# farhiongit/aho-corasick-1975

Hardware: AMD Instinct MI355X
Metric: input GB/s scanned, 1k-keyword dictionary, bit-exact match set (higher is better)
Workload: dtype u8; 1 GPU; BASELINE configs[1]: 1000 ASCII keywords, 1024 MiB synthetic text per GPU (1073741824 symbols of 1 B), 1 keyword planted per 4096 symbols; states=6492, lmax=12, matches_per_gpu=555000, matches_total=555000, parallelism=text sharded x1, 0-symbol halo (the largest any rank used), tables replicated

## Files before the change

aho-corasick-1975_amd/csrc/dev_gram2.h:

```cpp
constexpr uint32_t G2_STAGE = WAVE * 16 + 16;
constexpr uint32_t G2_LIST = 128;
constexpr uint32_t G2_Q2 = 64;
constexpr uint32_t G2_WAVE_BYTES = G2_STAGE + G2_LIST * 2 + G2_Q2 * 8;
static_assert (G2_WAVE_BYTES % 16 == 0, "the staged text is written 16 bytes per lane");
constexpr uint32_t G2_LDS_FIXED = (SPARSE_THREADS / WAVE) * G2_WAVE_BYTES + WALK_CTX_BYTES;

__device__ __forceinline__ uint32_t
wave_incl_scan_dpp (uint32_t v) {
  v += (uint32_t)__builtin_amdgcn_update_dpp (0, (int)v, 0x111, 0xf, 0xf, false);
  v += (uint32_t)__builtin_amdgcn_update_dpp (0, (int)v, 0x112, 0xf, 0xf, false);
  v += (uint32_t)__builtin_amdgcn_update_dpp (0, (int)v, 0x114, 0xf, 0xf, false);
  v += (uint32_t)__builtin_amdgcn_update_dpp (0, (int)v, 0x118, 0xf, 0xf, false);
  v += (uint32_t)__builtin_amdgcn_update_dpp (0, (int)v, 0x142, 0xa, 0xf, false);
  v += (uint32_t)__builtin_amdgcn_update_dpp (0, (int)v, 0x143, 0xc, 0xf, false);
  return v;
}

template <bool COUNT_ONLY, bool TILED>
__global__ __launch_bounds__ (SPARSE_THREADS) void
scan_gram2_kernel (GramK K, EmitCtx E, Launch A, const unsigned char *__restrict__ text, uint2 *items, uint32_t region_items,
                   uint32_t *fill, RecHole *holes, uint32_t resume, TileEntry *dir, uint32_t dir_base) {
  (void)items;
  (void)region_items;
  (void)fill;
  extern __shared__ __attribute__ ((aligned (16))) unsigned char smem[];
  constexpr uint32_t WAVES = SPARSE_THREADS / WAVE;
  constexpr uint32_t GROUP = WAVE * 16;
  {
    uint4 *dst = reinterpret_cast<uint4 *> (smem);
    const uint4 *src = reinterpret_cast<const uint4 *> (K.tab2);
    for (uint32_t i = threadIdx.x; i < (K.tab2_words + 3) / 4; i += blockDim.x)
      dst[i] = src[i];
  }
  uint32_t *next_tile = reinterpret_cast<uint32_t *> (smem + K.g2_off + WAVES * G2_WAVE_BYTES);
  StartsK *Ks = reinterpret_cast<StartsK *> (next_tile + 4);
  EmitCtx *Es = reinterpret_cast<EmitCtx *> (reinterpret_cast<unsigned char *> (Ks) + WALK_CTX_K);
  WaveRec *Ws = reinterpret_cast<WaveRec *> (reinterpret_cast<unsigned char *> (Ks) + WALK_CTX_K + WALK_CTX_E);
  if (threadIdx.x == 0) {
    *next_tile = 0;
    StartsK Kc{};
    Kc.srec = K.srec;
    Kc.sedge = K.sedge;
    Kc.remap = K.g4gid;
    Kc.remap_base = K.d5_begin;
    Kc.peek = K.g5peek;
    Kc.peek_packed = K.peek_packed;
    Kc.peek_rel = K.d5_rel;
    Kc.lo = K.lo;
    Kc.span = K.span;
    *Ks = Kc;
    *Es = E;
  }
  __syncthreads ();

  const uint32_t lane = threadIdx.x & (WAVE - 1);
  const uint32_t wib = uniform (threadIdx.x / WAVE);
  const uint32_t stage_off = K.g2_off + wib * G2_WAVE_BYTES;
  const uint32_t list_off = stage_off + G2_STAGE;
  uint2 *q2 = reinterpret_cast<uint2 *> (smem + stage_off + G2_STAGE + G2_LIST * 2);
  const uint32_t wave_id = blockIdx.x * WAVES + wib;
  uint2 *hits = reinterpret_cast<uint2 *> (Ws + wib);
  if (lane == 0) {
    WaveRec w0{};
    if (resume && !COUNT_ONLY && holes) {
      const RecHole h = holes[wave_id];
      if (h.len) {
        const unsigned long long at = ((unsigned long long)h.start_hi << 32) | h.start_lo;
        const unsigned long long base = at + h.len - E.rec_chunk;
        const bool below = base + E.rec_chunk <= E.capacity;
        const bool above = base >= E.capacity && base - E.capacity + E.rec_chunk <= E.spill_slots;
        const uint64_t dst = below ? reinterpret_cast<uint64_t> (&E.records[base]) : (above ? reinterpret_cast<uint64_t> (E.spill + (base - E.capacity)) : 0ull);
        w0.dst_lo = (uint32_t)dst;
        w0.dst_hi = (uint32_t)(dst >> 32);
        w0.base_lo = (uint32_t)base;
        w0.base_hi = (uint32_t)(base >> 32);
        w0.limit = (below || above) ? E.rec_chunk : 0u;
        w0.have = 1;
        w0.pad[0] = E.rec_chunk - h.len;
        w0.pad[1] = 1;
        w0.prev1 = w0.prev2 = NONE;
      }
    }
    if (!w0.have)
      w0.prev1 = w0.prev2 = NONE;
    Ws[wib] = w0;
  }
  const TileShare share (A);
  const uint32_t last_blk = (A.n - 1) / 16;
  uint32_t qn2 = 0;
  unsigned long long counted = 0;
  RecState rs = { 0ull, 0u };
  if (!COUNT_ONLY && resume) {
    rs = rec_state_load (hits);
    counted = uniform (reinterpret_cast<const WaveRec *> (hits)->pad[0]);
  }
  uint32_t it_x = 0, it_y = 0, pk = 0;
  uint2 pend_item = make_uint2 (0, 0), pend_e = make_uint2 (0, 0);
  uint32_t pend_r = 0, pend_n = 0;
  constexpr uint32_t PEND_NEED = 0x80000000u;
  auto lds_word = [&] (uint32_t byte_off) -> uint32_t {
    return *reinterpret_cast<const __attribute__ ((address_space (3))) uint32_t *> (byte_off);
  };
  const uint4 *text16 = reinterpret_cast<const uint4 *> (text);
  auto load_group = [&] (uint32_t g) -> uint4 {
    const uint32_t blk = g * WAVE + lane;
    typedef uint32_t nt_u32x4 __attribute__ ((ext_vector_type (4)));
    const nt_u32x4 v = __builtin_nontemporal_load (reinterpret_cast<const nt_u32x4 *> (text16) + (blk < last_blk ? blk : last_blk));
    return make_uint4 (v.x, v.y, v.z, v.w);
  };
  DIAG (const unsigned long long d_t0 = __builtin_readcyclecounter (); unsigned long long d_top = 0, d_sieve = 0, d_take = 0, d_cwait = 0, d_cons = 0, d_walk = 0, d_steps = 0;)
  auto walk_batch = [&] (uint32_t n_items) {
    DIAG (const unsigned long long d_wk = __builtin_readcyclecounter ();)
    const unsigned long long r = walk_starts<uint8_t, COUNT_ONLY, 2> (Ks, Es, text, q2, qn2, n_items, hits, counted);
    qn2 = uniform ((uint32_t)(r >> 32));
    counted = (uint32_t)r;
    if (!COUNT_ONLY)
      rs = rec_state_load (hits);
    DIAG (d_walk += __builtin_readcyclecounter () - d_wk;)
  };
  uint32_t peek_pos = 0, peek_cls = 0, peek_val = 0, peek_n = 0;
  const bool peek_inline = !COUNT_ONLY && K.peek_packed && K.d5_rel;
  auto push_walk = [&] (bool go, uint32_t ix, uint32_t iy) {
    const uint64_t m = __ballot (go);
    if (m) {
      while (qn2 + (uint32_t)__popcll (m) > G2_Q2)
        walk_batch (qn2 < WAVE ? qn2 : WAVE);
      if (go)
        q2[qn2 + rank_below (m)] = make_uint2 (ix, iy);
      qn2 = uniform (qn2 + (uint32_t)__popcll (m));
#if defined(ACM_GRAM2_ABLATE) && ACM_GRAM2_ABLATE == 2
      qn2 = 0;
#endif
      while (qn2 >= WAVE)
        walk_batch (WAVE);
    }
  };
  auto resolve_peeks = [&] () {
    if (peek_n == 0)
      return;
    const uint32_t ev = peek_val, cls = peek_cls & 31u;
    const uint32_t sym = (ev >> 31) ? GRAM_NO_PEEK : (ev >> 23) & 0xFFu;
    const uint32_t c1 = cls < K.span ? K.lo + cls : 0x100u;
    const bool on = (peek_cls >> 31) != 0 && (sym == GRAM_NO_PEEK || sym == c1);
    peek_n = 0;
    push_walk (on, peek_pos, (ev & 0x7FFFFFu) | WI_RECORD | cls << 24);
  };
  auto consume_pending = [&] () {
    if (pend_n == 0)
      return;
    DIAG (const unsigned long long d_c0 = __builtin_readcyclecounter (); asm volatile ("s_waitcnt vmcnt(0)" ::: "memory"); const unsigned long long d_c1 = __builtin_readcyclecounter (); d_cwait += d_c1 - d_c0; d_steps++; const unsigned long long d_w0 = d_walk;)
    struct { uint32_t x, y; } e = { pend_e.x, pend_e.y };
    const bool valid = lane < pend_n && (pend_r & PEND_NEED) != 0;
    const uint32_t r = pend_r & 0xFFu;
#if defined(ACM_GRAM2_ABLATE) && (ACM_GRAM2_ABLATE == 3 || ACM_GRAM2_ABLATE == 8)
    asm volatile ("" :: "v"(e.x), "v"(e.y));
    pend_n = 0;
    return;
#endif
    const bool far = valid && r >= 7 && (e.x & 0x20000000u) != 0;
    if (__ballot (far)) {
      const uint2 o = K.over2[far ? (e.x & 0x1FFFFFFFu) + (r - 7) : 0u];
      e.x = far ? o.x : e.x;
      e.y = far ? o.y : e.y;
    }
    if (!valid)
      e.x = 0;
    const bool at_record = (e.x & 0x40000000u) != 0;
#if !(defined(ACM_GRAM2_ABLATE) && ACM_GRAM2_ABLATE == 1)
    emit_terminals<COUNT_ONLY, true> (E, (e.x >> 31) != 0 && !at_record && pend_item.x + 3 >= E.emit_from, pend_item.x + 3, e.y, 4u, lane, hits, counted, Es, &rs);
    if (!COUNT_ONLY)
      counted = uniform ((uint32_t)counted);
#endif
    const uint32_t c4 = (pend_item.y >> 20) & 31u, c5 = (pend_item.y >> 25) & 31u;
    const bool child = ((e.x >> c4) & 1u) != 0 && !at_record;
    const uint32_t st5 = e.y + __popc (e.x & ((1u << c4) - 1u));
    if (peek_inline) {
      resolve_peeks ();
      uint32_t pv = 0;
      if (child)
        pv = K.g5peek[st5 - K.d5_begin];
      peek_val = pv;
      peek_pos = pend_item.x + 4;
      peek_cls = c5 | (child ? 0x80000000u : 0u);
      peek_n = __ballot (child) != 0 ? 1u : 0u;
      push_walk (at_record, pend_item.x + 3, e.y | WI_RECORD | c4 << 24);
    } else
      push_walk (child || at_record, at_record ? pend_item.x + 3 : pend_item.x + 4,
                 at_record ? e.y | WI_RECORD | (K.d5_rel ? c4 << 24 : 0u) : (K.d5_rel ? (st5 - K.d5_begin) | c5 << 24 : st5));
    pend_n = 0;
    DIAG (d_cons += (__builtin_readcyclecounter () - d_c1) - (d_walk - d_w0);)
  };
  auto batch_step = [&] (uint32_t n_items) {
    const uint32_t idx = it_y & 0xFFFFFu;
    const uint32_t word = lds_word ((idx >> 4) * 4u);
    consume_pending ();
    const uint32_t sh = (idx & 15u) * 2u;
    const bool need = lane < n_items && ((word >> sh) & 1u) != 0;
    const uint32_t r = __popc (word & 0x55555555u & ((1u << sh) - 1u));
    uint2 e = make_uint2 (0, 0);
#if defined(ACM_GRAM2_ABLATE) && ACM_GRAM2_ABLATE == 8
    if (need)
      e = K.rows2[r < 7 ? r : 7];
#else
    if (need)
      e = K.rows2[(size_t)(idx >> 4) * 8 + (r < 7 ? r : 7)];
#endif
    pend_e = e;
    pend_item = make_uint2 (it_x, it_y);
    pend_r = r | (need ? PEND_NEED : 0u);
    pend_n = n_items;
  };

  auto sieve_group = [&] (const uint4 cur, const uint32_t next_x, const uint32_t next_y, const uint32_t g, uint4 &prefetched, uint32_t &pass_out, uint32_t &my_out) -> uint32_t {
    typedef uint32_t u32x4 __attribute__ ((ext_vector_type (4)));
    typedef uint32_t u32x2 __attribute__ ((ext_vector_type (2)));
    uint32_t t4 = (uint32_t)__builtin_amdgcn_update_dpp ((int)uniform (next_x), (int)cur.x, 0x130, 0xf, 0xf, false);
    const uint32_t t5 = (uint32_t)__builtin_amdgcn_update_dpp ((int)uniform (next_y), (int)cur.y, 0x130, 0xf, 0xf, false);
    asm volatile ("" : "+v"(t4));
    __builtin_amdgcn_sched_barrier (0);
    prefetched = load_group (g + 4);
    const uint32_t t0 = cur.x, t1 = cur.y, t2 = cur.z, t3 = cur.w;
    *reinterpret_cast<__attribute__ ((address_space (3))) u32x4 *> (stage_off + lane * 16u) = u32x4{ t0, t1, t2, t3 };
    if (lane == WAVE - 1)
      *reinterpret_cast<__attribute__ ((address_space (3))) u32x2 *> (stage_off + GROUP) = u32x2{ t4, t5 };
    const uint32_t pos0 = g * GROUP + lane * 16;
    const uint32_t w[5] = { t0, t1, t2, t3, t4 };
#if defined(ACM_GRAM2_ABLATE) && ACM_GRAM2_ABLATE == 7
    asm volatile ("" :: "v"(w[0]), "v"(w[1]), "v"(w[2]), "v"(w[3]), "v"(w[4]));
    pass_out = 0;
    return 0;
#endif
    uint32_t c[20];
#pragma unroll
    for (int j = 0; j < 20; j++) {
      const uint32_t b = (w[j / 4] >> (8 * (j % 4))) & 0xFFu;
      c[j] = min (b - K.lo, K.span);
    }
    if (__builtin_expect (uniform (g * GROUP + GROUP + 20) > A.n, 0)) {
#pragma unroll
      for (int j = 0; j < 20; j++)
        if (pos0 + j >= A.n)
          c[j] = K.span;
    }
    uint32_t pair[19];
#pragma unroll
    for (int j = 0; j < 19; j++)
      pair[j] = __umul24 (c[j], K.W) + c[j + 1];
    const uint32_t W2 = K.W * K.W;
    uint32_t acc = 0;
#pragma unroll
    for (int h = 0; h < 2; h++) {
      uint32_t ix[8], word[8];
#pragma unroll
      for (int j = 0; j < 8; j++) {
        ix[j] = __umul24 (pair[8 * h + j], W2) + pair[8 * h + j + 2];
        word[j] = lds_word ((ix[j] >> 4) * 4u);
      }
#pragma unroll
      for (int j = 0; j < 8; j++)
        acc |= __builtin_amdgcn_ubfe (word[j], ix[j] << 1, 2u) << (2 * (8 * h + j));
    }
    const uint32_t ix16 = __umul24 (pair[16], W2) + pair[18];
    const uint32_t h16 = __builtin_amdgcn_ubfe (lds_word ((ix16 >> 4) * 4u), (ix16 << 1) | 1u, 1u);
    const uint32_t pass = acc & ((acc >> 1) | (acc >> 3) | (h16 << 30)) & 0x55555555u;
    pass_out = pass;
#if defined(ACM_GRAM2_ABLATE) && ACM_GRAM2_ABLATE == 6
    asm volatile ("" :: "v"(pass));
    return 0;
#endif
    const uint32_t cnt = __popc (pass);
    const uint32_t incl = wave_incl_scan_dpp (cnt);
    my_out = incl - cnt;
    return (uint32_t)__builtin_amdgcn_readlane ((int)incl, WAVE - 1);
  };
  auto take_group = [&] (const uint32_t g, const uint32_t total, uint32_t pass, uint32_t my) {
    const uint32_t W2 = K.W * K.W;
    const bool tail = g * GROUP + GROUP + 8 > A.n;
    for (uint32_t base = 0; base < total; base += G2_LIST) {
      const uint32_t n_here = total - base < G2_LIST ? total - base : G2_LIST;
      {
        const uint32_t lim = base + n_here;
        while (pass != 0 && my < lim) {
          const uint32_t b = (uint32_t)__builtin_ctz (pass);
          *reinterpret_cast<__attribute__ ((address_space (3))) uint16_t *> (list_off + (my - base) * 2u) = (uint16_t)(lane * 16u + (b >> 1));
          pass &= pass - 1u;
          my++;
        }
      }
#if defined(ACM_GRAM2_ABLATE) && ACM_GRAM2_ABLATE == 5
      continue;
#endif
      for (uint32_t off = 0; off < n_here;) {
        const uint32_t take = n_here - off < WAVE - pk ? n_here - off : WAVE - pk;
        const bool mine = lane >= pk && lane < pk + take;
        const uint32_t li = mine ? off + lane - pk : 0u;
        const uint32_t q = *reinterpret_cast<const __attribute__ ((address_space (3))) uint16_t *> (list_off + li * 2u);
        const uint32_t a = stage_off + (q & ~3u);
        const uint32_t d0 = lds_word (a), d1 = lds_word (a + 4u), d2 = lds_word (a + 8u);
        const uint32_t lo4 = __builtin_amdgcn_alignbyte (d1, d0, q), hi4 = __builtin_amdgcn_alignbyte (d2, d1, q);
        uint32_t r[6];
#pragma unroll
        for (int k = 0; k < 6; k++) {
          const uint32_t b = ((k < 4 ? lo4 : hi4) >> (8 * (k % 4))) & 0xFFu;
          r[k] = min (b - K.lo, K.span);
        }
        const uint32_t p = g * GROUP + q;
        if (tail) {
#pragma unroll
          for (int k = 0; k < 6; k++)
            if (p + k >= A.n)
              r[k] = K.span;
        }
        const uint32_t idx = __umul24 (__umul24 (r[0], K.W) + r[1], W2) + __umul24 (r[2], K.W) + r[3];
        const uint32_t y = idx | (r[4] << 20) | (r[5] << 25);
        it_x = mine ? p : it_x;
        it_y = mine ? y : it_y;
        pk += take;
        off += take;
#if defined(ACM_GRAM2_ABLATE) && ACM_GRAM2_ABLATE == 4
        if (pk == WAVE) {
          asm volatile ("" :: "v"(it_x), "v"(it_y));
          pk = 0;
        }
        continue;
#endif
        if (pk == WAVE) {
          batch_step (WAVE);
          pk = 0;
        }
      }
    }
  };

  static_assert (!TILED || !COUNT_ONLY, "tiled scans write their records themselves");
  constexpr bool tiled = TILED;
  auto stream_index = [&] (const WaveRec &w) -> uint32_t { return w.have ? (w.pad[1] - 1u) * REC_CHUNK + (uint32_t)counted : 0u; };
  if (tiled && lane == 0)
    Ws[wib].tile = NONE;
  auto drain = [&] () {
    if (pk) {
      batch_step (pk);
      pk = 0;
    }
    consume_pending ();
    resolve_peeks ();
    while (qn2)
      walk_batch (qn2 < WAVE ? qn2 : WAVE);
  };
  for (;;) {
    const uint32_t tile = share.next (next_tile, lane);
    if (tiled) {
      drain ();
      if (lane == 0) {
        const WaveRec w = Ws[wib];
        if (w.tile != NONE) {
          const uint32_t s_end = stream_index (w), cur_tile = w.tile;
          const uint32_t tile_begin = cur_tile * K.R * GROUP, tile_len = K.R * GROUP;
          const uint32_t tile_end = A.n - tile_begin < tile_len ? A.n : tile_begin + tile_len;
          TileEntry e;
          e.end_slot = w.have ? (((unsigned long long)w.base_hi << 32) | w.base_lo) + (uint32_t)counted : 0ull;
          e.lo = E.pos_base + (tile_begin > E.emit_from ? tile_begin : E.emit_from);
          e.hi = E.pos_base + tile_end;
          e.n = s_end - w.s_begin;
          e.n_late = s_end - w.s_late;
          e.c1 = w.prev1;
          e.c2 = w.prev1 != NONE ? w.prev2 : NONE;
          e.pad[0] = e.pad[1] = 0;
          dir[dir_base + (cur_tile - A.range_begin)] = e;
        }
      }
    }
    if (tile == NONE)
      break;
    if (tiled && lane == 0) {
      WaveRec *W = Ws + wib;
      W->tile = tile;
      W->s_begin = W->s_late = stream_index (*W);
    }
    const uint32_t g0 = tile * K.R;
    uint4 c0 = load_group (g0), c1 = load_group (g0 + 1), c2 = load_group (g0 + 2), c3 = load_group (g0 + 3);
    for (uint32_t k = 0; k < K.R; k++) {
      if (tiled && k + 1 == K.R && lane == 0)
        Ws[wib].s_late = stream_index (Ws[wib]);
      uint4 n3;
      uint32_t pass = 0, my = 0;
      DIAG (const unsigned long long d_g0 = __builtin_readcyclecounter (); asm volatile ("s_waitcnt vmcnt(0)" ::: "memory"); const unsigned long long d_g1 = __builtin_readcyclecounter (); d_top += d_g1 - d_g0;)
      const uint32_t total = sieve_group (c0, c1.x, c1.y, g0 + k, n3, pass, my);
      DIAG (const unsigned long long d_g2 = __builtin_readcyclecounter (); d_sieve += d_g2 - d_g1; const unsigned long long d_in = d_cwait + d_cons + d_walk;)
      if (total)
        take_group (g0 + k, total, pass, my);
      DIAG (d_take += (__builtin_readcyclecounter () - d_g2) - (d_cwait + d_cons + d_walk - d_in);)
      c0 = c1;
      c1 = c2;
      c2 = c3;
      c3 = n3;
    }
  }
  if (!tiled)
    drain ();
  DIAG (if (lane == 0 && wave_id < 8192) {
    unsigned long long *o = g_acm_diag[wave_id];
    o[0] = __builtin_readcyclecounter () - d_t0;
    o[1] = d_top;
    o[2] = d_sieve;
    o[3] = d_take;
    o[4] = d_cwait;
    o[5] = d_cons;
    o[6] = d_walk;
    o[7] = d_steps;
  })
  if (COUNT_ONLY) {
    const uint32_t incl = wave_incl_scan ((uint32_t)counted);
    const uint32_t total = __shfl (incl, WAVE - 1, WAVE);
    if (lane == 0 && total)
      atomicAdd (E.count, (unsigned long long)total);
  } else {
    if (lane == 0 && holes) {
      const WaveRec w = Ws[wib];
      const unsigned long long at = (((unsigned long long)w.base_hi << 32) | w.base_lo) + (uint32_t)counted;
      RecHole h = { (uint32_t)at, (uint32_t)(at >> 32), w.have ? E.rec_chunk - (uint32_t)counted : 0u, 0u };
      holes[wave_id] = h;
    }
  }
}
```

Baseline: 3853 GB/s.

## Unroll sieve loop by four with rotating registers and move prefetch after sieve math

```diff
diff --git a/aho-corasick-1975_amd/csrc/dev_gram2.h b/aho-corasick-1975_amd/csrc/dev_gram2.h
--- a/aho-corasick-1975_amd/csrc/dev_gram2.h
+++ b/aho-corasick-1975_amd/csrc/dev_gram2.h
@@ -14,6 +14,13 @@
   v += (uint32_t)__builtin_amdgcn_update_dpp (0, (int)v, 0x142, 0xa, 0xf, false);
   v += (uint32_t)__builtin_amdgcn_update_dpp (0, (int)v, 0x143, 0xc, 0xf, false);
   return v;
+}
+
+__device__ __forceinline__ uint32_t
+mad24 (uint32_t a, uint32_t s, uint32_t c) {
+  uint32_t d;
+  asm ("v_mad_u32_u24 %0, %1, %2, %3" : "=v"(d) : "v"(a), "s"(s), "v"(c));
+  return d;
 }
 
 template <bool COUNT_ONLY, bool TILED>
@@ -98,18 +105,18 @@
   uint2 pend_item = make_uint2 (0, 0), pend_e = make_uint2 (0, 0);
   uint32_t pend_r = 0, pend_n = 0;
   constexpr uint32_t PEND_NEED = 0x80000000u;
-  auto lds_word = [&] (uint32_t byte_off) -> uint32_t {
+  auto lds_word = [&] (uint32_t byte_off) __attribute__ ((always_inline)) -> uint32_t {
     return *reinterpret_cast<const __attribute__ ((address_space (3))) uint32_t *> (byte_off);
   };
   const uint4 *text16 = reinterpret_cast<const uint4 *> (text);
-  auto load_group = [&] (uint32_t g) -> uint4 {
+  auto load_group = [&] (uint32_t g) __attribute__ ((always_inline)) -> uint4 {
     const uint32_t blk = g * WAVE + lane;
     typedef uint32_t nt_u32x4 __attribute__ ((ext_vector_type (4)));
     const nt_u32x4 v = __builtin_nontemporal_load (reinterpret_cast<const nt_u32x4 *> (text16) + (blk < last_blk ? blk : last_blk));
     return make_uint4 (v.x, v.y, v.z, v.w);
   };
   DIAG (const unsigned long long d_t0 = __builtin_readcyclecounter (); unsigned long long d_top = 0, d_sieve = 0, d_take = 0, d_cwait = 0, d_cons = 0, d_walk = 0, d_steps = 0;)
-  auto walk_batch = [&] (uint32_t n_items) {
+  auto walk_batch = [&] (uint32_t n_items) __attribute__ ((always_inline)) {
     DIAG (const unsigned long long d_wk = __builtin_readcyclecounter ();)
     const unsigned long long r = walk_starts<uint8_t, COUNT_ONLY, 2> (Ks, Es, text, q2, qn2, n_items, hits, counted);
     qn2 = uniform ((uint32_t)(r >> 32));
@@ -120,7 +127,7 @@
   };
   uint32_t peek_pos = 0, peek_cls = 0, peek_val = 0, peek_n = 0;
   const bool peek_inline = !COUNT_ONLY && K.peek_packed && K.d5_rel;
-  auto push_walk = [&] (bool go, uint32_t ix, uint32_t iy) {
+  auto push_walk = [&] (bool go, uint32_t ix, uint32_t iy) __attribute__ ((always_inline)) {
     const uint64_t m = __ballot (go);
     if (m) {
       while (qn2 + (uint32_t)__popcll (m) > G2_Q2)
@@ -135,7 +142,7 @@
         walk_batch (WAVE);
     }
   };
-  auto resolve_peeks = [&] () {
+  auto resolve_peeks = [&] () __attribute__ ((always_inline)) {
     if (peek_n == 0)
       return;
     const uint32_t ev = peek_val, cls = peek_cls & 31u;
@@ -145,7 +152,7 @@
     peek_n = 0;
     push_walk (on, peek_pos, (ev & 0x7FFFFFu) | WI_RECORD | cls << 24);
   };
-  auto consume_pending = [&] () {
+  auto consume_pending = [&] () __attribute__ ((always_inline)) {
     if (pend_n == 0)
       return;
     DIAG (const unsigned long long d_c0 = __builtin_readcyclecounter (); asm volatile ("s_waitcnt vmcnt(0)" ::: "memory"); const unsigned long long d_c1 = __builtin_readcyclecounter (); d_cwait += d_c1 - d_c0; d_steps++; const unsigned long long d_w0 = d_walk;)
@@ -190,7 +197,7 @@
     pend_n = 0;
     DIAG (d_cons += (__builtin_readcyclecounter () - d_c1) - (d_walk - d_w0);)
   };
-  auto batch_step = [&] (uint32_t n_items) {
+  auto batch_step = [&] (uint32_t n_items) __attribute__ ((always_inline)) {
     const uint32_t idx = it_y & 0xFFFFFu;
     const uint32_t word = lds_word ((idx >> 4) * 4u);
     consume_pending ();
@@ -211,14 +218,11 @@
     pend_n = n_items;
   };
 
-  auto sieve_group = [&] (const uint4 cur, const uint32_t next_x, const uint32_t next_y, const uint32_t g, uint4 &prefetched, uint32_t &pass_out, uint32_t &my_out) -> uint32_t {
+  auto sieve_group = [&] (const uint4 cur, const uint32_t next_x, const uint32_t next_y, const uint32_t g, uint4 &prefetched, uint32_t &pass_out, uint32_t &my_out) __attribute__ ((always_inline)) -> uint32_t {
     typedef uint32_t u32x4 __attribute__ ((ext_vector_type (4)));
     typedef uint32_t u32x2 __attribute__ ((ext_vector_type (2)));
     uint32_t t4 = (uint32_t)__builtin_amdgcn_update_dpp ((int)uniform (next_x), (int)cur.x, 0x130, 0xf, 0xf, false);
     const uint32_t t5 = (uint32_t)__builtin_amdgcn_update_dpp ((int)uniform (next_y), (int)cur.y, 0x130, 0xf, 0xf, false);
-    asm volatile ("" : "+v"(t4));
-    __builtin_amdgcn_sched_barrier (0);
-    prefetched = load_group (g + 4);
     const uint32_t t0 = cur.x, t1 = cur.y, t2 = cur.z, t3 = cur.w;
     *reinterpret_cast<__attribute__ ((address_space (3))) u32x4 *> (stage_off + lane * 16u) = u32x4{ t0, t1, t2, t3 };
     if (lane == WAVE - 1)
@@ -227,6 +231,7 @@
     const uint32_t w[5] = { t0, t1, t2, t3, t4 };
 #if defined(ACM_GRAM2_ABLATE) && ACM_GRAM2_ABLATE == 7
     asm volatile ("" :: "v"(w[0]), "v"(w[1]), "v"(w[2]), "v"(w[3]), "v"(w[4]));
+    prefetched = load_group (g + 4);
     pass_out = 0;
     return 0;
 #endif
@@ -242,10 +247,13 @@
         if (pos0 + j >= A.n)
           c[j] = K.span;
     }
+    __builtin_amdgcn_sched_barrier (0);
+    prefetched = load_group (g + 4);
+    __builtin_amdgcn_sched_barrier (0);
     uint32_t pair[19];
 #pragma unroll
     for (int j = 0; j < 19; j++)
-      pair[j] = __umul24 (c[j], K.W) + c[j + 1];
+      pair[j] = mad24 (c[j], K.W, c[j + 1]);
     const uint32_t W2 = K.W * K.W;
     uint32_t acc = 0;
 #pragma unroll
@@ -253,14 +261,16 @@
       uint32_t ix[8], word[8];
 #pragma unroll
       for (int j = 0; j < 8; j++) {
-        ix[j] = __umul24 (pair[8 * h + j], W2) + pair[8 * h + j + 2];
+        ix[j] = mad24 (pair[8 * h + j], W2, pair[8 * h + j + 2]);
         word[j] = lds_word ((ix[j] >> 4) * 4u);
       }
 #pragma unroll
-      for (int j = 0; j < 8; j++)
+      for (int j = 0; j < 8; j++) {
         acc |= __builtin_amdgcn_ubfe (word[j], ix[j] << 1, 2u) << (2 * (8 * h + j));
-    }
-    const uint32_t ix16 = __umul24 (pair[16], W2) + pair[18];
+        asm ("" : "+v"(acc));
+      }
+    }
+    const uint32_t ix16 = mad24 (pair[16], W2, pair[18]);
     const uint32_t h16 = __builtin_amdgcn_ubfe (lds_word ((ix16 >> 4) * 4u), (ix16 << 1) | 1u, 1u);
     const uint32_t pass = acc & ((acc >> 1) | (acc >> 3) | (h16 << 30)) & 0x55555555u;
     pass_out = pass;
@@ -273,28 +283,30 @@
     my_out = incl - cnt;
     return (uint32_t)__builtin_amdgcn_readlane ((int)incl, WAVE - 1);
   };
-  auto take_group = [&] (const uint32_t g, const uint32_t total, uint32_t pass, uint32_t my) {
+  auto take_group = [&] (const uint32_t g, const uint32_t total, uint32_t pass, uint32_t my) __attribute__ ((always_inline)) {
     const uint32_t W2 = K.W * K.W;
     const bool tail = g * GROUP + GROUP + 8 > A.n;
-    for (uint32_t base = 0; base < total; base += G2_LIST) {
+    uint32_t wa = list_off + my * 2u;
+    for (uint32_t base = 0; base < total; base += G2_LIST, wa -= G2_LIST * 2u) {
       const uint32_t n_here = total - base < G2_LIST ? total - base : G2_LIST;
       {
-        const uint32_t lim = base + n_here;
-        while (pass != 0 && my < lim) {
+        const uint32_t wend = list_off + n_here * 2u;
+        while (pass != 0 && wa < wend) {
           const uint32_t b = (uint32_t)__builtin_ctz (pass);
-          *reinterpret_cast<__attribute__ ((address_space (3))) uint16_t *> (list_off + (my - base) * 2u) = (uint16_t)(lane * 16u + (b >> 1));
+          *reinterpret_cast<__attribute__ ((address_space (3))) uint16_t *> (wa) = (uint16_t)(lane * 32u + b);
           pass &= pass - 1u;
-          my++;
+          wa += 2u;
         }
       }
 #if defined(ACM_GRAM2_ABLATE) && ACM_GRAM2_ABLATE == 5
       continue;
 #endif
-      for (uint32_t off = 0; off < n_here;) {
-        const uint32_t take = n_here - off < WAVE - pk ? n_here - off : WAVE - pk;
-        const bool mine = lane >= pk && lane < pk + take;
-        const uint32_t li = mine ? off + lane - pk : 0u;
-        const uint32_t q = *reinterpret_cast<const __attribute__ ((address_space (3))) uint16_t *> (list_off + li * 2u);
+      for (uint32_t off = 0; off < n_here; off += WAVE) {
+        const uint32_t take = n_here - off < WAVE ? n_here - off : WAVE;
+        const uint32_t j = (lane - pk) & (WAVE - 1);
+        const bool mine = j < take;
+        const uint32_t li = mine ? off + j : 0u;
+        const uint32_t q = *reinterpret_cast<const __attribute__ ((address_space (3))) uint16_t *> (list_off + li * 2u) >> 1;
         const uint32_t a = stage_off + (q & ~3u);
         const uint32_t d0 = lds_word (a), d1 = lds_word (a + 4u), d2 = lds_word (a + 8u);
         const uint32_t lo4 = __builtin_amdgcn_alignbyte (d1, d0, q), hi4 = __builtin_amdgcn_alignbyte (d2, d1, q);
@@ -311,23 +323,24 @@
             if (p + k >= A.n)
               r[k] = K.span;
         }
-        const uint32_t idx = __umul24 (__umul24 (r[0], K.W) + r[1], W2) + __umul24 (r[2], K.W) + r[3];
+        const uint32_t idx = mad24 (mad24 (r[0], K.W, r[1]), W2, mad24 (r[2], K.W, r[3]));
         const uint32_t y = idx | (r[4] << 20) | (r[5] << 25);
-        it_x = mine ? p : it_x;
-        it_y = mine ? y : it_y;
-        pk += take;
-        off += take;
+        const bool first = mine && lane >= pk;
+        it_x = first ? p : it_x;
+        it_y = first ? y : it_y;
+        if (pk + take < WAVE) {
+          pk += take;
+          continue;
+        }
 #if defined(ACM_GRAM2_ABLATE) && ACM_GRAM2_ABLATE == 4
-        if (pk == WAVE) {
-          asm volatile ("" :: "v"(it_x), "v"(it_y));
-          pk = 0;
-        }
-        continue;
-#endif
-        if (pk == WAVE) {
-          batch_step (WAVE);
-          pk = 0;
-        }
+        asm volatile ("" :: "v"(it_x), "v"(it_y));
+#else
+        batch_step (WAVE);
+#endif
+        const bool second = mine && lane < pk;
+        it_x = second ? p : it_x;
+        it_y = second ? y : it_y;
+        pk = pk + take - WAVE;
       }
     }
   };
@@ -379,17 +392,27 @@
     }
     const uint32_t g0 = tile * K.R;
     uint4 c0 = load_group (g0), c1 = load_group (g0 + 1), c2 = load_group (g0 + 2), c3 = load_group (g0 + 3);
-    for (uint32_t k = 0; k < K.R; k++) {
+    auto one_group = [&] (uint4 &set, const uint4 &behind, const uint32_t k) __attribute__ ((always_inline)) {
       if (tiled && k + 1 == K.R && lane == 0)
         Ws[wib].s_late = stream_index (Ws[wib]);
-      uint4 n3;
       uint32_t pass = 0, my = 0;
       DIAG (const unsigned long long d_g0 = __builtin_readcyclecounter (); asm volatile ("s_waitcnt vmcnt(0)" ::: "memory"); const unsigned long long d_g1 = __builtin_readcyclecounter (); d_top += d_g1 - d_g0;)
-      const uint32_t total = sieve_group (c0, c1.x, c1.y, g0 + k, n3, pass, my);
+      const uint32_t total = sieve_group (set, behind.x, behind.y, g0 + k, set, pass, my);
       DIAG (const unsigned long long d_g2 = __builtin_readcyclecounter (); d_sieve += d_g2 - d_g1; const unsigned long long d_in = d_cwait + d_cons + d_walk;)
       if (total)
         take_group (g0 + k, total, pass, my);
       DIAG (d_take += (__builtin_readcyclecounter () - d_g2) - (d_cwait + d_cons + d_walk - d_in);)
+    };
+    uint32_t k = 0;
+    for (; k + 4 <= K.R; k += 4) {
+      one_group (c0, c1, k);
+      one_group (c1, c2, k + 1);
+      one_group (c2, c3, k + 2);
+      one_group (c3, c0, k + 3);
+    }
+    for (; k < K.R; k++) {
+      one_group (c0, c1, k);
+      const uint4 n3 = c0;
       c0 = c1;
       c1 = c2;
       c2 = c3;
```

New measurement: 3848 GB/s. About the same (-0.1%).
